# hustvl/4DGaussians

Hardware: NVIDIA H100
Metric: render FPS @300k gauss 1352x1014 (fused deform+rasterize forward); train-step ms in `train_step` (higher is better)
Workload: dtype f32

## Files before the change

### 4dgaussians_b200/csrc/g4d_deform_tc.cu

```cuda
#include "geom_finish.cuh"
#include "tc_wgmma.cuh"

namespace g4d {

template <int ARITH> struct TcArith;
template <> struct TcArith<2> {
    static constexpr int KS = 16, ES = 2, EPC = 8, NWG = 2, PH = 1;
    static constexpr float SF = 64.f, SA = 8.f, SW = 256.f;
};
template <> struct TcArith<1> {
    static constexpr int KS = 8, ES = 4, EPC = 4, NWG = 1, PH = 4;
    static constexpr float SF = 1.f, SA = 1.f, SW = 1.f;
};
constexpr float kF16Max = 65504.f;
constexpr int kStageCols = 60;
constexpr uint32_t kMaxSmemPerBlock = 227u * 1024u;
constexpr uint32_t kTcStaticSmem = (uint32_t)((sizeof(CameraDev) + 127) & ~(size_t)127);

struct TcSmem { uint32_t w1, w0, w2, bias, w2s, stage, bars, part_bytes, total; };

inline TcSmem tc_smem_layout(int arith, int F, bool sh) {
    const uint32_t es = arith == 2 ? 2u : 4u, ph = arith == 2 ? 1u : 4u, nwg = arith == 2 ? 2u : 1u;
    TcSmem s{};
    uint32_t off = 0;
    auto take = [&](uint32_t bytes) { uint32_t o = off; off += (bytes + 127u) & ~127u; return o; };
    s.part_bytes = 2u * 128u * (128u / ph) * es;
    s.w1 = take(2u * s.part_bytes);
    s.w0 = take(2u * 128u * F * es);
    s.w2 = take(sh ? 2u * 48u * 128u * es : 128u);
    s.bias = take((128 + G4D_NUM_HEADS * 128 + 64) * 4);
    s.w2s = take(4 * 128 * 16);
    s.stage = take(nwg * 64u * kStageCols * 4u);
    s.bars = take(64);
    s.total = off;
    return s;
}

struct TcPackDesc {
    const float* src[1 + G4D_NUM_HEADS + 1];
    uint8_t* dst[1 + G4D_NUM_HEADS + 1];
    int rows[1 + G4D_NUM_HEADS + 1], K[1 + G4D_NUM_HEADS + 1], parts[1 + G4D_NUM_HEADS + 1], kperm[1 + G4D_NUM_HEADS + 1];
    int start[2 + G4D_NUM_HEADS + 1];
    int count, arith;
    uint32_t* status;
};

__global__ void tc_pack_weights_kernel(TcPackDesc p) {
    const int i = blockIdx.x * blockDim.x + threadIdx.x;
    if (i >= p.start[p.count]) return;
    int m = 0;
    while (i >= p.start[m + 1]) ++m;
    const int e = i - p.start[m];
    const uint32_t K = (uint32_t)p.K[m], n = (uint32_t)e / K, k = (uint32_t)e % K, rows = (uint32_t)p.rows[m];
    const uint32_t kd = p.kperm[m] ? wg::tf32_kperm(k) : k;
    const uint32_t KP = K / (uint32_t)p.parts[m], part = kd / KP, kk = kd % KP;
    const float v = __ldg(p.src[m] + e);
    if (p.arith == 2) {
        uint32_t hi, lo;
        if (fabsf(v * TcArith<2>::SW) >= kF16Max && p.status) *reinterpret_cast<volatile uint32_t*>(p.status) = 1u;
        wg::f16_split2(v * TcArith<2>::SW, 0.f, hi, lo);
        uint8_t* base = p.dst[m] + (size_t)part * 2u * rows * KP * 2u + wg::img16_off(n, kk, KP);
        *reinterpret_cast<uint16_t*>(base) = (uint16_t)hi;
        *reinterpret_cast<uint16_t*>(base + rows * KP * 2u) = (uint16_t)lo;
    } else {
        uint32_t hi, lo;
        wg::tf32_split(v, hi, lo);
        uint8_t* base = p.dst[m] + (size_t)part * 2u * rows * KP * 4u + wg::img32_off(n, kk, KP);
        *reinterpret_cast<uint32_t*>(base) = hi;
        *reinterpret_cast<uint32_t*>(base + rows * KP * 4u) = lo;
    }
}

size_t tc_packed_floats(const G4DDeformParams& prm) {
    const int F = prm.levels * prm.channels;
    size_t f = 2 * (size_t)128 * F;
    for (int h = 0; h < G4D_NUM_HEADS; ++h) f += 2 * (size_t)128 * 128 + (h == 4 ? 2 * (size_t)48 * 128 : 0);
    return f + 64;
}

cudaError_t launch_tc_pack_weights(const G4DDeformParams& prm, int arith, float* blob, TcWeights* out, cudaStream_t st) {
    TcPackDesc p{};
    p.arith = arith;
    p.status = out->status;
    const int F = prm.levels * prm.channels;
    const size_t es = arith == 2 ? 2 : 4;
    int m = 0, total = 0;
    uint8_t* q = reinterpret_cast<uint8_t*>(blob);
    auto add = [&](const float* src, int rows, int K, int parts, int kperm) {
        p.src[m] = src; p.dst[m] = q; p.rows[m] = rows; p.K[m] = K; p.parts[m] = parts; p.kperm[m] = kperm && arith == 1;
        p.start[m] = total;
        total += rows * K;
        uint8_t* r = q;
        q += 2 * (size_t)rows * K * es;
        ++m;
        return reinterpret_cast<const float*>(r);
    };
    out->w0 = add(prm.w0, 128, F, 1, 0);
    for (int h = 0; h < G4D_NUM_HEADS; ++h) {
        out->w1[h] = nullptr; out->w2[h] = nullptr;
        if (!(prm.head_mask & (1 << h))) continue;
        out->w1[h] = add(prm.w1[h], 128, 128, arith == 2 ? TcArith<2>::PH : TcArith<1>::PH, 1);
        if (h == 4) out->w2[h] = add(prm.w2[h], 48, 128, 1, 1);
    }
    p.start[m] = total; p.count = m;
    tc_pack_weights_kernel<<<(total + 255) / 256, 256, 0, st>>>(p);
    return cudaGetLastError();
}

__device__ __forceinline__ float4 sample_vector(const DeformDesc* __restrict__ dp, int l, int v, int C4, float px, float py, float pz) {
    const DeformDesc& d = *dp;
    const float pcs[3] = {px, py, pz};
    Tap1D tx[3];
#pragma unroll
    for (int a = 0; a < 3; ++a) tx[a] = make_tap(pcs[a], d.res[l][a]);
    float4 prod = make_float4(1.f, 1.f, 1.f, 1.f);
#pragma unroll
    for (int k = 0; k < 6; ++k) {
        const int c0 = plane_axis0(k), c1 = plane_axis1(k);
        float4 s;
        if (c1 == 3) {
            const float4* rowp = reinterpret_cast<const float4*>(d.trow[l][c0]);
            const float4 r0 = __ldg(rowp + tx[c0].i0 * C4 + v), r1 = __ldg(rowp + tx[c0].i1 * C4 + v);
            const float w0 = tx[c0].w0, w1 = tx[c0].w1;
            s.x = fmaf(r1.x, w1, r0.x * w0); s.y = fmaf(r1.y, w1, r0.y * w0);
            s.z = fmaf(r1.z, w1, r0.z * w0); s.w = fmaf(r1.w, w1, r0.w * w0);
        } else {
            const int W = d.res[l][c0];
            const float4* pl = reinterpret_cast<const float4*>(d.planes[l][k]);
            const Tap1D &X = tx[c0], &Y = tx[c1];
            const float4 nw = __ldg(pl + (Y.i0 * W + X.i0) * C4 + v), ne = __ldg(pl + (Y.i0 * W + X.i1) * C4 + v);
            const float4 sw = __ldg(pl + (Y.i1 * W + X.i0) * C4 + v), se = __ldg(pl + (Y.i1 * W + X.i1) * C4 + v);
            const float wnw = X.w0 * Y.w0, wne = X.w1 * Y.w0, wsw = X.w0 * Y.w1, wse = X.w1 * Y.w1;
            s.x = fmaf(se.x, wse, fmaf(sw.x, wsw, fmaf(ne.x, wne, nw.x * wnw)));
            s.y = fmaf(se.y, wse, fmaf(sw.y, wsw, fmaf(ne.y, wne, nw.y * wnw)));
            s.z = fmaf(se.z, wse, fmaf(sw.z, wsw, fmaf(ne.z, wne, nw.z * wnw)));
            s.w = fmaf(se.w, wse, fmaf(sw.w, wsw, fmaf(ne.w, wne, nw.w * wnw)));
        }
        prod.x *= s.x; prod.y *= s.y; prod.z *= s.z; prod.w *= s.w;
    }
    return prod;
}


using wg::Frags;

template <int ARITH, int NS>
__device__ __forceinline__ void put_block(Frags<NS>& a, int j, float x0, float x1, float y0, float y1) {
    if constexpr (ARITH == 2) {
        const int s = j >> 1, o = (j & 1) * 2;
        wg::f16_split2(x0, x1, a.hi[s][o], a.lo[s][o]);
        wg::f16_split2(y0, y1, a.hi[s][o + 1], a.lo[s][o + 1]);
    } else {
        wg::tf32_split(x0, a.hi[j][0], a.lo[j][0]);
        wg::tf32_split(y0, a.hi[j][1], a.lo[j][1]);
        wg::tf32_split(x1, a.hi[j][2], a.lo[j][2]);
        wg::tf32_split(y1, a.hi[j][3], a.lo[j][3]);
    }
}

template <int ARITH, int N, int NS, int NSP>
__device__ __forceinline__ void gemm3(float (&d)[N / 2], const Frags<NS>& a, int s0, uint32_t b_hi, uint32_t b_lo, uint32_t bcols,
                                      bool accumulate) {
    using A = TcArith<ARITH>;
    const uint64_t dh = wg::desc_kmajor(b_hi, bcols, A::EPC), dl = wg::desc_kmajor(b_lo, bcols, A::EPC);
    wg::fence_regs(d);
    wg::fence();
#pragma unroll
    for (int p = 0; p < 3; ++p) {
#pragma unroll
        for (int s = 0; s < NSP; ++s) {
            const uint64_t bd = ((p == 1) ? dl : dh) + (uint64_t)(16 * s);
            const uint32_t acc = (accumulate || p > 0 || s > 0) ? 1u : 0u;
            if constexpr (ARITH == 2) wg::mma_f16_rs<N, 0>(d, p == 0 ? a.lo[s0 + s] : a.hi[s0 + s], bd, acc);
            else wg::mma_tf32_rs<N>(d, p == 0 ? a.lo[s0 + s] : a.hi[s0 + s], bd, acc);
        }
    }
    wg::commit();
    wg::wait_all();
    wg::fence_regs(d);
}

template <int ARITH>
__device__ __forceinline__ void relu_to_frags(const float (&d)[64], float inv, const float* __restrict__ bias, int t, Frags<128 / TcArith<ARITH>::KS>& a,
                                              uint32_t (&b0)[4], uint32_t (&b1)[4], float& mx) {
#pragma unroll
    for (int w = 0; w < 4; ++w) { b0[w] = 0u; b1[w] = 0u; }
#pragma unroll
    for (int j = 0; j < 16; ++j) {
        const int c = 8 * j + 2 * t;
        const float2 bb = *reinterpret_cast<const float2*>(bias + c);
        const float x0 = fmaf(d[4 * j], inv, bb.x), x1 = fmaf(d[4 * j + 1], inv, bb.y);
        const float y0 = fmaf(d[4 * j + 2], inv, bb.x), y1 = fmaf(d[4 * j + 3], inv, bb.y);
        const int sh = 8 * (j & 3) + 2 * t;
        b0[j >> 2] |= ((x0 > 0.f ? 1u : 0u) | (x1 > 0.f ? 2u : 0u)) << sh;
        b1[j >> 2] |= ((y0 > 0.f ? 1u : 0u) | (y1 > 0.f ? 2u : 0u)) << sh;
        const float r0 = fmaxf(x0, 0.f), r1 = fmaxf(x1, 0.f), r2 = fmaxf(y0, 0.f), r3 = fmaxf(y1, 0.f);
        mx = fmaxf(mx, fmaxf(fmaxf(r0, r1), fmaxf(r2, r3)));
        put_block<ARITH>(a, j, r0, r1, r2, r3);
    }
#pragma unroll
    for (int w = 0; w < 4; ++w) {
        b0[w] |= __shfl_xor_sync(0xffffffffu, b0[w], 1); b0[w] |= __shfl_xor_sync(0xffffffffu, b0[w], 2);
        b1[w] |= __shfl_xor_sync(0xffffffffu, b1[w], 1); b1[w] |= __shfl_xor_sync(0xffffffffu, b1[w], 2);
    }
}

__device__ __forceinline__ void store_bits(uint32_t* base, int slot, int64_t n, int64_t g0, int64_t g1, int t, const uint32_t (&b0)[4],
                                           const uint32_t (&b1)[4]) {
    const uint32_t w0 = t == 0 ? b0[0] : t == 1 ? b0[1] : t == 2 ? b0[2] : b0[3];
    const uint32_t w1 = t == 0 ? b1[0] : t == 1 ? b1[1] : t == 2 ? b1[2] : b1[3];
    if (g0 < n) base[((size_t)slot * (size_t)n + (size_t)g0) * 4 + t] = w0;
    if (g1 < n) base[((size_t)slot * (size_t)n + (size_t)g1) * 4 + t] = w1;
}

__device__ __forceinline__ void mbar_arrive(void* bar) {
    asm volatile("mbarrier.arrive.shared::cta.b64 _, [%0];" ::"r"(smem_u32(bar)) : "memory");
}
__device__ __forceinline__ void bar_sync(int id, int count) { asm volatile("bar.sync %0, %1;" ::"r"(id), "r"(count) : "memory"); }

template <int ARITH, int MODE, int C, int L, bool SAVE>
__global__ void __launch_bounds__(TcArith<ARITH>::NWG * 128, 1)
deform_tc_kernel(DeformDesc d, TcWeights tw, TcSmem Ls, const CameraDev* __restrict__ camp, int use_cam, int64_t n, DeformIO io) {
    using A = TcArith<ARITH>;
    constexpr int F = C * L, NS0 = F / A::KS, NS1 = 128 / A::KS, NSP = NS1 / A::PH, TM = 64 * A::NWG, NT = 128 * A::NWG;
    static_assert(F % 16 == 0 && F <= 64, "feature width must be 32, 48 or 64");
    constexpr float kInvL0 = A::SA / (A::SF * A::SW), kInvH = 1.f / (A::SA * A::SW), kInvHS = 1.f / A::SW;
    extern __shared__ __align__(128) uint8_t smem[];
    __shared__ CameraDev cam;
    const int tid = threadIdx.x, wgi = tid >> 7, t128 = tid & 127, lane = tid & 31, g = lane >> 2, t = lane & 3;
    const int r0 = ((t128 >> 5) << 4) + g, r1 = r0 + 8;
    float* sBias = reinterpret_cast<float*>(smem + Ls.bias);
    float4* sW2s = reinterpret_cast<float4*>(smem + Ls.w2s);
    float* stage = reinterpret_cast<float*>(smem + Ls.stage) + wgi * 64 * kStageCols;
    uint64_t* bars = reinterpret_cast<uint64_t*>(smem + Ls.bars);
    uint64_t *bar_w0 = bars, *bar_full = bars + 1, *bar_empty = bars + 3;
    for (int i = tid; i < 128; i += NT) sBias[i] = __ldg(d.b0 + i) * A::SA;
    for (int i = tid; i < 64; i += NT) sBias[128 + G4D_NUM_HEADS * 128 + i] = 0.f;
    for (int h = 0; h < G4D_NUM_HEADS; ++h) {
        if (!(d.head_mask & (1 << h))) continue;
        for (int i = tid; i < 128; i += NT) sBias[128 + h * 128 + i] = __ldg(d.b1[h] + i) * (h == 4 ? A::SA : 1.f);
        if (h < 4) {
            const int ko = head_out(h);
            for (int j = tid; j < 128; j += NT)
                sW2s[h * 128 + j] = make_float4(__ldg(d.w2[h] + j), ko > 1 ? __ldg(d.w2[h] + 128 + j) : 0.f,
                                               ko > 2 ? __ldg(d.w2[h] + 256 + j) : 0.f, ko > 3 ? __ldg(d.w2[h] + 384 + j) : 0.f);
        }
    }
    __syncthreads();
    for (int h = 0; h < G4D_NUM_HEADS; ++h) {
        if (!(d.head_mask & (1 << h))) continue;
        for (int i = tid; i < head_out(h); i += NT) sBias[128 + G4D_NUM_HEADS * 128 + (h < 4 ? 4 * h : 16) + i] = __ldg(d.b2[h] + i);
    }
    if (tid == 0) {
        mbar_init(bar_w0, 1);
        mbar_init(bar_full, 1); mbar_init(bar_full + 1, 1);
        mbar_init(bar_empty, 4 * A::NWG); mbar_init(bar_empty + 1, 4 * A::NWG);
        fence_barrier_init();
    }
    pdl_wait();
    pdl_trigger();
    if (use_cam) {
        for (int i = tid; i < (int)(sizeof(CameraDev) / 4); i += NT)
            reinterpret_cast<uint32_t*>(&cam)[i] = reinterpret_cast<const uint32_t*>(camp)[i];
    }
    __syncthreads();

    const bool hsh = d.head_mask & G4D_HEAD_SHS;
    const int m_heads = __popc(d.head_mask & 31);
    uint32_t hseq = 0;
    {
        int k = 0;
        for (int h = 0; h < G4D_NUM_HEADS; ++h)
            if (d.head_mask & (1 << h)) hseq |= (uint32_t)h << (3 * k++);
    }
    const int64_t ntiles = (n + TM - 1) / TM;
    const int64_t my_tiles = (int64_t)blockIdx.x < ntiles ? (ntiles - 1 - blockIdx.x) / gridDim.x + 1 : 0;
    const uint32_t per_tile = (uint32_t)(m_heads * A::PH), total_items = (uint32_t)my_tiles * per_tile;
    auto issue = [&](uint32_t u) {
        const uint32_t s = u & 1u, r = u % per_tile;
        if (u >= 2) mbar_wait(bar_empty + s, ((u >> 1) - 1u) & 1u);
        const int h = (int)((hseq >> (3 * (r / A::PH))) & 7u);
        mbar_expect_tx(bar_full + s, Ls.part_bytes);
        tma_bulk_g2s(smem + Ls.w1 + s * Ls.part_bytes, reinterpret_cast<const uint8_t*>(tw.w1[h]) + (r % A::PH) * Ls.part_bytes,
                     Ls.part_bytes, bar_full + s);
    };
    if (tid == 0) {
        const uint32_t w0b = 2u * 128u * F * A::ES, w2b = hsh ? 2u * 48u * 128u * A::ES : 0u;
        mbar_expect_tx(bar_w0, w0b + w2b);
        tma_bulk_g2s(smem + Ls.w0, tw.w0, w0b, bar_w0);
        if (hsh) tma_bulk_g2s(smem + Ls.w2, tw.w2[4], w2b, bar_w0);
        if (total_items) issue(0);
    }
    __syncwarp();
    mbar_wait(bar_w0, 0);
    const uint32_t sW0 = wg::smem_addr(smem + Ls.w0), sW1 = wg::smem_addr(smem + Ls.w1), sW2 = wg::smem_addr(smem + Ls.w2);
    const float* b2s = sBias + 128 + G4D_NUM_HEADS * 128;
    float mx = 0.f;
    uint32_t u = 0;
    const bool dbg = tw.dbg && tid == 0;
    const long long t_start = dbg ? clock64() : 0;
    long long t_wait = 0;

    for (int64_t it = 0; it < my_tiles; ++it) {
        const int64_t tile = (int64_t)blockIdx.x + it * gridDim.x;
        const int64_t row0 = tile * TM + wgi * 64, g0 = row0 + r0, g1 = row0 + r1;
        float acc[64];
        {
            Frags<NS0> x;
            const float* f0 = tw.feat + g0 * F;
            const float* f1 = tw.feat + g1 * F;
#pragma unroll
            for (int s = 0; s < NS0; ++s) {
                float v[8];
#pragma unroll
                for (int hlf = 0; hlf < 2; ++hlf) {
                    const int c = ARITH == 2 ? 16 * s + 8 * hlf + 2 * t : 8 * s + 4 * hlf + t;
                    if (ARITH == 2) {
                        const float2 p0 = g0 < n ? __ldg(reinterpret_cast<const float2*>(f0 + c)) : make_float2(0.f, 0.f);
                        const float2 p1 = g1 < n ? __ldg(reinterpret_cast<const float2*>(f1 + c)) : make_float2(0.f, 0.f);
                        v[4 * hlf] = p0.x * A::SF; v[4 * hlf + 1] = p0.y * A::SF; v[4 * hlf + 2] = p1.x * A::SF; v[4 * hlf + 3] = p1.y * A::SF;
                    } else {
                        v[4 * hlf] = g0 < n ? __ldg(f0 + c) : 0.f;
                        v[4 * hlf + 2] = g1 < n ? __ldg(f1 + c) : 0.f;
                    }
                }
                if (ARITH == 2) {
#pragma unroll
                    for (int e = 0; e < 8; ++e) mx = fmaxf(mx, fabsf(v[e]));
                    wg::f16_split2(v[0], v[1], x.hi[s][0], x.lo[s][0]);
                    wg::f16_split2(v[2], v[3], x.hi[s][1], x.lo[s][1]);
                    wg::f16_split2(v[4], v[5], x.hi[s][2], x.lo[s][2]);
                    wg::f16_split2(v[6], v[7], x.hi[s][3], x.lo[s][3]);
                } else {
                    wg::tf32_split(v[0], x.hi[s][0], x.lo[s][0]);
                    wg::tf32_split(v[2], x.hi[s][1], x.lo[s][1]);
                    wg::tf32_split(v[4], x.hi[s][2], x.lo[s][2]);
                    wg::tf32_split(v[6], x.hi[s][3], x.lo[s][3]);
                }
            }
            gemm3<ARITH, 128, NS0, NS0>(acc, x, 0, sW0, sW0 + 128u * F * A::ES, F, false);
        }
        Frags<NS1> a1;
        {
            uint32_t bw0[4], bw1[4];
            relu_to_frags<ARITH>(acc, kInvL0, sBias, t, a1, bw0, bw1, mx);
            if (SAVE) store_bits(tw.relu_bits, 0, n, g0, g1, t, bw0, bw1);
        }
        if (t == 0) {
#pragma unroll
            for (int j = 0; j < 11; ++j) { stage[r0 * kStageCols + j] = 0.f; stage[r1 * kStageCols + j] = 0.f; }
        }
#pragma unroll 1
        for (int k = 0; k < m_heads; ++k) {
            const int h = (int)((hseq >> (3 * k)) & 7u);
#pragma unroll 1
            for (int p = 0; p < A::PH; ++p, ++u) {
                if (tid == 0 && u + 1 < total_items) issue(u + 1);
                __syncwarp();
                const uint32_t s = u & 1u;
                const long long t0 = dbg ? clock64() : 0;
                mbar_wait(bar_full + s, (u >> 1) & 1u);
                if (dbg) t_wait += clock64() - t0;
                const uint32_t b = sW1 + s * Ls.part_bytes;
                if constexpr (A::PH == 1) {
                    gemm3<ARITH, 128, NS1, NSP>(acc, a1, 0, b, b + Ls.part_bytes / 2, 128 / A::PH, false);
                } else {
#pragma unroll
                    for (int pp = 0; pp < A::PH; ++pp)
                        if (pp == p) gemm3<ARITH, 128, NS1, NSP>(acc, a1, pp * NSP, b, b + Ls.part_bytes / 2, 128 / A::PH, pp != 0);
                }
                if (lane == 0) mbar_arrive(bar_empty + s);
            }
            uint32_t bw0[4], bw1[4];
            if (h < 4) {
                const float* b1 = sBias + 128 + h * 128;
                const float4* w2 = sW2s + h * 128;
                float o0[4] = {0.f, 0.f, 0.f, 0.f}, o1[4] = {0.f, 0.f, 0.f, 0.f};
#pragma unroll
                for (int w = 0; w < 4; ++w) { bw0[w] = 0u; bw1[w] = 0u; }
#pragma unroll
                for (int j = 0; j < 16; ++j) {
                    const int c = 8 * j + 2 * t;
                    const float2 bb = *reinterpret_cast<const float2*>(b1 + c);
                    const float x0 = fmaf(acc[4 * j], kInvH, bb.x), x1 = fmaf(acc[4 * j + 1], kInvH, bb.y);
                    const float y0 = fmaf(acc[4 * j + 2], kInvH, bb.x), y1 = fmaf(acc[4 * j + 3], kInvH, bb.y);
                    const int sh = 8 * (j & 3) + 2 * t;
                    bw0[j >> 2] |= ((x0 > 0.f ? 1u : 0u) | (x1 > 0.f ? 2u : 0u)) << sh;
                    bw1[j >> 2] |= ((y0 > 0.f ? 1u : 0u) | (y1 > 0.f ? 2u : 0u)) << sh;
                    const float4 wa = w2[c], wb = w2[c + 1];
                    const float ax = fmaxf(x0, 0.f), ay = fmaxf(x1, 0.f), bx = fmaxf(y0, 0.f), by = fmaxf(y1, 0.f);
                    o0[0] = fmaf(ay, wb.x, fmaf(ax, wa.x, o0[0])); o0[1] = fmaf(ay, wb.y, fmaf(ax, wa.y, o0[1]));
                    o0[2] = fmaf(ay, wb.z, fmaf(ax, wa.z, o0[2])); o0[3] = fmaf(ay, wb.w, fmaf(ax, wa.w, o0[3]));
                    o1[0] = fmaf(by, wb.x, fmaf(bx, wa.x, o1[0])); o1[1] = fmaf(by, wb.y, fmaf(bx, wa.y, o1[1]));
                    o1[2] = fmaf(by, wb.z, fmaf(bx, wa.z, o1[2])); o1[3] = fmaf(by, wb.w, fmaf(bx, wa.w, o1[3]));
                }
#pragma unroll
                for (int o = 0; o < 4; ++o) {
                    o0[o] += __shfl_xor_sync(0xffffffffu, o0[o], 1); o0[o] += __shfl_xor_sync(0xffffffffu, o0[o], 2);
                    o1[o] += __shfl_xor_sync(0xffffffffu, o1[o], 1); o1[o] += __shfl_xor_sync(0xffffffffu, o1[o], 2);
                }
#pragma unroll
                for (int w = 0; w < 4; ++w) {
                    bw0[w] |= __shfl_xor_sync(0xffffffffu, bw0[w], 1); bw0[w] |= __shfl_xor_sync(0xffffffffu, bw0[w], 2);
                    bw1[w] |= __shfl_xor_sync(0xffffffffu, bw1[w], 1); bw1[w] |= __shfl_xor_sync(0xffffffffu, bw1[w], 2);
                }
                if (t == 0) {
                    const int ko = head_out(h), col = head_col(h);
#pragma unroll
                    for (int o = 0; o < 4; ++o) {
                        if (o < ko) {
                            stage[r0 * kStageCols + col + o] = o0[o] + b2s[4 * h + o];
                            stage[r1 * kStageCols + col + o] = o1[o] + b2s[4 * h + o];
                        }
                    }
                }
            } else {
                relu_to_frags<ARITH>(acc, kInvHS, sBias + 128 + 4 * 128, t, a1, bw0, bw1, mx);
                float acc2[24];
                gemm3<ARITH, 48, NS1, NS1>(acc2, a1, 0, sW2, sW2 + 48u * 128u * A::ES, 128, false);
                const float* b2sh = b2s + 16;
#pragma unroll
                for (int j = 0; j < 6; ++j) {
                    const int c = 8 * j + 2 * t;
                    stage[r0 * kStageCols + 11 + c] = fmaf(acc2[4 * j], kInvH, b2sh[c]);
                    stage[r0 * kStageCols + 12 + c] = fmaf(acc2[4 * j + 1], kInvH, b2sh[c + 1]);
                    stage[r1 * kStageCols + 11 + c] = fmaf(acc2[4 * j + 2], kInvH, b2sh[c]);
                    stage[r1 * kStageCols + 12 + c] = fmaf(acc2[4 * j + 3], kInvH, b2sh[c + 1]);
                }
            }
            if (SAVE) store_bits(tw.relu_bits, 1 + h, n, g0, g1, t, bw0, bw1);
        }
        bar_sync(1 + wgi, 128);
        {
            const int row = t128 & 63;
            const int64_t gi = row0 + row;
            const float* o = stage + row * kStageCols;
            if (gi < n) {
                const Vec3 p{io.xyz[3 * gi] + o[0], io.xyz[3 * gi + 1] + o[1], io.xyz[3 * gi + 2] + o[2]};
                if (t128 < 64) {
                    float sl[3] = {0.f, 0.f, 0.f}, q[4] = {0.f, 0.f, 0.f, 0.f}, ol = 0.f;
                    if (io.scaling) { sl[0] = io.scaling[3 * gi]; sl[1] = io.scaling[3 * gi + 1]; sl[2] = io.scaling[3 * gi + 2]; }
                    if (io.rotation) { const float4 r4 = *reinterpret_cast<const float4*>(io.rotation + 4 * gi); q[0] = r4.x; q[1] = r4.y; q[2] = r4.z; q[3] = r4.w; }
                    if (io.opacity) ol = io.opacity[gi];
                    sl[0] += o[3]; sl[1] += o[4]; sl[2] += o[5];
                    q[0] += o[6]; q[1] += o[7]; q[2] += o[8]; q[3] += o[9];
                    ol += o[10];
                    if (MODE == 0) {
                        io.out_xyz[3 * gi] = p.x; io.out_xyz[3 * gi + 1] = p.y; io.out_xyz[3 * gi + 2] = p.z;
                        if (io.out_scaling) { io.out_scaling[3 * gi] = sl[0]; io.out_scaling[3 * gi + 1] = sl[1]; io.out_scaling[3 * gi + 2] = sl[2]; }
                        if (io.out_rotation) *reinterpret_cast<float4*>(io.out_rotation + 4 * gi) = make_float4(q[0], q[1], q[2], q[3]);
                        if (io.out_opacity) io.out_opacity[gi] = ol;
                    } else {
                        fused_finish_geometry(cam, io, gi, p, sl, q, ol);
                    }
                } else {
                    float dsh[48];
#pragma unroll
                    for (int j = 0; j < 48; ++j) dsh[j] = hsh ? o[11 + j] : 0.f;
                    if (MODE == 0) {
                        if (io.out_shs && hsh) {
#pragma unroll
                            for (int j = 0; j < 48; j += 4) {
                                const float4 b = *reinterpret_cast<const float4*>(io.shs + gi * 48 + j);
                                *reinterpret_cast<float4*>(io.out_shs + gi * 48 + j) = make_float4(b.x + dsh[j], b.y + dsh[j + 1], b.z + dsh[j + 2], b.w + dsh[j + 3]);
                            }
                        }
                    } else {
                        fused_finish_colour(cam, io, gi, p, hsh, dsh);
                    }
                }
            }
        }
        bar_sync(1 + wgi, 128);
    }
    if (ARITH == 2 && mx >= kF16Max && tw.status) *reinterpret_cast<volatile uint32_t*>(tw.status) = 1u;
    if (dbg) { tw.dbg[blockIdx.x * 12] = clock64() - t_start; tw.dbg[blockIdx.x * 12 + 1] = t_wait; }
}

template <int C4>
__global__ void __launch_bounds__(256) deform_features_kernel(DeformDesc d, int64_t n, const float* __restrict__ xyz, float* __restrict__ feat) {
    pdl_wait();
    pdl_trigger();
    const int64_t t = (int64_t)blockIdx.x * 256 + threadIdx.x;
    const int64_t g = t / C4;
    const int v = (int)(t % C4);
    if (g >= n) return;
    float pcs[3];
#pragma unroll
    for (int a = 0; a < 3; ++a) {
        const float amax = __ldg(d.aabb + a), ascale = 2.0f / (__ldg(d.aabb + 3 + a) - amax);
        pcs[a] = (xyz[3 * g + a] - amax) * ascale - 1.0f;
    }
    for (int l = 0; l < d.levels; ++l)
        *reinterpret_cast<float4*>(feat + g * d.F + l * d.C + 4 * v) = sample_vector(&d, l, v, C4, pcs[0], pcs[1], pcs[2]);
}

cudaError_t launch_deform_features(const DeformDesc& d, int64_t n, const float* xyz, float* feat, cudaStream_t st) {
    if (n == 0) return cudaSuccess;
    const int C4 = d.C / 4;
    const unsigned grid = (unsigned)((n * C4 + 255) / 256);
    if (C4 == 4) return launch_k(deform_features_kernel<4>, dim3(grid), dim3(256), 0, st, true, d, n, xyz, feat);
    if (C4 == 8) return launch_k(deform_features_kernel<8>, dim3(grid), dim3(256), 0, st, true, d, n, xyz, feat);
    return cudaErrorInvalidValue;
}

bool tc_deform_supported(const DeformDesc& d, int arith) {
    if (d.WD != 128) return false;
    if (!((d.C == 16 && (d.levels == 2 || d.levels == 3)) || (d.C == 32 && d.levels == 2))) return false;
    return tc_smem_layout(arith, d.F, (d.head_mask & G4D_HEAD_SHS) != 0).total + kTcStaticSmem <= kMaxSmemPerBlock;
}

template <int ARITH, int MODE, int C, int L>
static cudaError_t launch_deform_tc_t(const DeformDesc& d, const TcWeights& tw, const TcSmem& Ls, size_t bytes, int grid,
                                      const CameraDev* cam, bool use_cam, int64_t n, const DeformIO& io, cudaStream_t st) {
    constexpr int threads = TcArith<ARITH>::NWG * 128;
    cudaError_t e;
    if (tw.relu_bits) {
        e = cudaFuncSetAttribute(deform_tc_kernel<ARITH, MODE, C, L, true>, cudaFuncAttributeMaxDynamicSharedMemorySize, (int)bytes);
        if (e != cudaSuccess) return e;
        return launch_k(deform_tc_kernel<ARITH, MODE, C, L, true>, dim3(grid), dim3(threads), bytes, st, true, d, tw, Ls, cam, use_cam ? 1 : 0, n, io);
    }
    e = cudaFuncSetAttribute(deform_tc_kernel<ARITH, MODE, C, L, false>, cudaFuncAttributeMaxDynamicSharedMemorySize, (int)bytes);
    if (e != cudaSuccess) return e;
    return launch_k(deform_tc_kernel<ARITH, MODE, C, L, false>, dim3(grid), dim3(threads), bytes, st, true, d, tw, Ls, cam, use_cam ? 1 : 0, n, io);
}

cudaError_t launch_deform_tc(const DeformDesc& d, const TcWeights& tw, int mode, const CameraDev* cam, bool use_cam_time,
                             int64_t n, const DeformIO& io, int sm_count, cudaStream_t st) {
    if (n == 0) return cudaSuccess;
    if (!tw.feat) return cudaErrorInvalidValue;
    {
        cudaError_t e = launch_deform_features(d, n, io.xyz, tw.feat, st);
        if (e != cudaSuccess) return e;
    }
    const TcSmem Ls = tc_smem_layout(tw.arith, d.F, (d.head_mask & G4D_HEAD_SHS) != 0);
    const size_t bytes = Ls.total;
    const int64_t ntiles = (n + 64 * (tw.arith == 2 ? 2 : 1) - 1) / (64 * (tw.arith == 2 ? 2 : 1));
    const int grid = (int)(ntiles < sm_count ? ntiles : sm_count);
    const bool use_cam = mode == 1 || use_cam_time;
#define G4D_TC_CASE(AR, CC, LL)                                                                                        \
    if (tw.arith == AR && d.C == CC && d.levels == LL)                                                                 \
        return mode == 0 ? launch_deform_tc_t<AR, 0, CC, LL>(d, tw, Ls, bytes, grid, cam, use_cam, n, io, st)          \
                         : launch_deform_tc_t<AR, 1, CC, LL>(d, tw, Ls, bytes, grid, cam, use_cam, n, io, st);
    G4D_TC_CASE(2, 16, 2)
    G4D_TC_CASE(2, 16, 3)
    G4D_TC_CASE(2, 32, 2)
    G4D_TC_CASE(1, 16, 2)
    G4D_TC_CASE(1, 16, 3)
    G4D_TC_CASE(1, 32, 2)
#undef G4D_TC_CASE
    return cudaErrorInvalidValue;
}

}
```

Baseline: 879.5.

## Alternate warpgroup tensor-core issue turns and prefetch next tile inputs into L2

Adds a ping-pong handshake between the two warpgroups, using named barriers around each wgmma issue, so their GEMM issue phases alternate and overlap one group's epilogue with the other's MMAs. The TMA issue for the next weight part is moved to after the MMA commit so it overlaps the in-flight GEMM. Thread 0 also issues bulk L2 prefetches of the next tile's per-gaussian inputs (xyz, scaling, rotation, opacity, SH). Debug timing is extended to more sections. The extra barriers add sync overhead and could serialize the warpgroups if the phases are not well balanced.

```diff
diff --git a/4dgaussians_b200/csrc/g4d_deform_tc.cu b/4dgaussians_b200/csrc/g4d_deform_tc.cu
--- a/4dgaussians_b200/csrc/g4d_deform_tc.cu
+++ b/4dgaussians_b200/csrc/g4d_deform_tc.cu
@@ -158,9 +158,9 @@
     }
 }
 
-template <int ARITH, int N, int NS, int NSP>
+template <int ARITH, int N, int NS, int NSP, class Queued>
 __device__ __forceinline__ void gemm3(float (&d)[N / 2], const Frags<NS>& a, int s0, uint32_t b_hi, uint32_t b_lo, uint32_t bcols,
-                                      bool accumulate) {
+                                      bool accumulate, Queued&& queued) {
     using A = TcArith<ARITH>;
     const uint64_t dh = wg::desc_kmajor(b_hi, bcols, A::EPC), dl = wg::desc_kmajor(b_lo, bcols, A::EPC);
     wg::fence_regs(d);
@@ -176,6 +176,7 @@
         }
     }
     wg::commit();
+    queued();
     wg::wait_all();
     wg::fence_regs(d);
 }
@@ -217,6 +218,12 @@
     asm volatile("mbarrier.arrive.shared::cta.b64 _, [%0];" ::"r"(smem_u32(bar)) : "memory");
 }
 __device__ __forceinline__ void bar_sync(int id, int count) { asm volatile("bar.sync %0, %1;" ::"r"(id), "r"(count) : "memory"); }
+__device__ __forceinline__ void bar_arrive(int id, int count) { asm volatile("bar.arrive %0, %1;" ::"r"(id), "r"(count) : "memory"); }
+__device__ __forceinline__ void prefetch_rows_l2(const float* base, int64_t g0, int64_t g1, int width) {
+    if (!base || g1 <= g0) return;
+    const uintptr_t a = ((uintptr_t)(base + g0 * width) + 15u) & ~(uintptr_t)15u, e = (uintptr_t)(base + g1 * width) & ~(uintptr_t)15u;
+    if (e > a) asm volatile("cp.async.bulk.prefetch.L2.global [%0], %1;" ::"l"(a), "r"((uint32_t)(e - a)) : "memory");
+}
 
 template <int ARITH, int MODE, int C, int L, bool SAVE>
 __global__ void __launch_bounds__(TcArith<ARITH>::NWG * 128, 1)
@@ -299,11 +306,32 @@
     uint32_t u = 0;
     const bool dbg = tw.dbg && tid == 0;
     const long long t_start = dbg ? clock64() : 0;
-    long long t_wait = 0;
+    auto note = [&](int k, long long t0) { if (dbg) tw.dbg[blockIdx.x * 12 + k] += clock64() - t0; };
+    uint32_t sections = 0;
+    auto turn_take = [&]() {
+        if constexpr (A::NWG == 2) {
+            if (wgi == 1 || sections > 0) {
+                const long long t0 = dbg ? clock64() : 0;
+                bar_sync(3 + wgi, 256);
+                note(3, t0);
+            }
+        }
+    };
+    auto turn_pass = [&]() {
+        if constexpr (A::NWG == 2) { bar_arrive(4 - wgi, 256); ++sections; }
+    };
 
     for (int64_t it = 0; it < my_tiles; ++it) {
         const int64_t tile = (int64_t)blockIdx.x + it * gridDim.x;
         const int64_t row0 = tile * TM + wgi * 64, g0 = row0 + r0, g1 = row0 + r1;
+        if (tid == 0 && it + 1 < my_tiles) {
+            const int64_t q0 = (tile + gridDim.x) * TM, q1 = q0 + TM < n ? q0 + TM : n;
+            prefetch_rows_l2(io.xyz, q0, q1, 3);
+            prefetch_rows_l2(io.scaling, q0, q1, 3);
+            prefetch_rows_l2(io.rotation, q0, q1, 4);
+            prefetch_rows_l2(io.opacity, q0, q1, 1);
+            prefetch_rows_l2(io.shs, q0, q1, 48);
+        }
         float acc[64];
         {
             Frags<NS0> x;
@@ -338,7 +366,8 @@
                     wg::tf32_split(v[6], x.hi[s][3], x.lo[s][3]);
                 }
             }
-            gemm3<ARITH, 128, NS0, NS0>(acc, x, 0, sW0, sW0 + 128u * F * A::ES, F, false);
+            turn_take();
+            gemm3<ARITH, 128, NS0, NS0>(acc, x, 0, sW0, sW0 + 128u * F * A::ES, F, false, turn_pass);
         }
         Frags<NS1> a1;
         {
@@ -355,19 +384,27 @@
             const int h = (int)((hseq >> (3 * k)) & 7u);
 #pragma unroll 1
             for (int p = 0; p < A::PH; ++p, ++u) {
-                if (tid == 0 && u + 1 < total_items) issue(u + 1);
-                __syncwarp();
                 const uint32_t s = u & 1u;
                 const long long t0 = dbg ? clock64() : 0;
                 mbar_wait(bar_full + s, (u >> 1) & 1u);
-                if (dbg) t_wait += clock64() - t0;
+                note(1, t0);
                 const uint32_t b = sW1 + s * Ls.part_bytes;
+                auto queued = [&]() {
+                    turn_pass();
+                    if (tid == 0 && u + 1 < total_items) {
+                        const long long t1 = dbg ? clock64() : 0;
+                        issue(u + 1);
+                        note(2, t1);
+                    }
+                    __syncwarp();
+                };
+                turn_take();
                 if constexpr (A::PH == 1) {
-                    gemm3<ARITH, 128, NS1, NSP>(acc, a1, 0, b, b + Ls.part_bytes / 2, 128 / A::PH, false);
+                    gemm3<ARITH, 128, NS1, NSP>(acc, a1, 0, b, b + Ls.part_bytes / 2, 128 / A::PH, false, queued);
                 } else {
 #pragma unroll
                     for (int pp = 0; pp < A::PH; ++pp)
-                        if (pp == p) gemm3<ARITH, 128, NS1, NSP>(acc, a1, pp * NSP, b, b + Ls.part_bytes / 2, 128 / A::PH, pp != 0);
+                        if (pp == p) gemm3<ARITH, 128, NS1, NSP>(acc, a1, pp * NSP, b, b + Ls.part_bytes / 2, 128 / A::PH, pp != 0, queued);
                 }
                 if (lane == 0) mbar_arrive(bar_empty + s);
             }
@@ -417,7 +454,8 @@
             } else {
                 relu_to_frags<ARITH>(acc, kInvHS, sBias + 128 + 4 * 128, t, a1, bw0, bw1, mx);
                 float acc2[24];
-                gemm3<ARITH, 48, NS1, NS1>(acc2, a1, 0, sW2, sW2 + 48u * 128u * A::ES, 128, false);
+                turn_take();
+                gemm3<ARITH, 48, NS1, NS1>(acc2, a1, 0, sW2, sW2 + 48u * 128u * A::ES, 128, false, turn_pass);
                 const float* b2sh = b2s + 16;
 #pragma unroll
                 for (int j = 0; j < 6; ++j) {
@@ -430,6 +468,7 @@
             }
             if (SAVE) store_bits(tw.relu_bits, 1 + h, n, g0, g1, t, bw0, bw1);
         }
+        const long long t_tail0 = dbg ? clock64() : 0;
         bar_sync(1 + wgi, 128);
         {
             const int row = t128 & 63;
@@ -472,9 +511,11 @@
             }
         }
         bar_sync(1 + wgi, 128);
-    }
+        note(4, t_tail0);
+    }
+    if (A::NWG == 2 && wgi == 0 && sections > 0) bar_sync(3, 256);
     if (ARITH == 2 && mx >= kF16Max && tw.status) *reinterpret_cast<volatile uint32_t*>(tw.status) = 1u;
-    if (dbg) { tw.dbg[blockIdx.x * 12] = clock64() - t_start; tw.dbg[blockIdx.x * 12 + 1] = t_wait; }
+    note(0, t_start);
 }
 
 template <int C4>
```

Result: no change. 886.2, median of 6 (+0.8%).
